# open-genome/dna

Measured on AMD Instinct MI355X. Metric: MLM sequences/sec, DNABERT-2-117M seq_len=512, at 1/2/4/8 MI355X, higher is better.
Workload: dtype bf16

## Files before the change

dna_amd/build.py:

```python
import argparse
import concurrent.futures as cf
import glob
import os
import shutil
import subprocess
import sys

HERE = os.path.dirname(os.path.abspath(__file__))
ROOT = os.path.dirname(HERE)
CSRC = os.path.join(HERE, "csrc")
INCLUDE = os.path.join(ROOT, "include")
BUILD = os.path.join(ROOT, "build", "native")
LIB = os.path.join(HERE, "lib", "libdna_amd.so")
ARCH = os.environ.get("DNA_AMD_ARCH", "gfx950")
HIPCC = os.environ.get("HIPCC", "/opt/rocm/bin/hipcc")

HIP_FLAGS = ["--offload-arch=" + ARCH, "-O3", "-fPIC", "-std=c++17", "-I", INCLUDE, "-I", CSRC,
             "-mllvm", "-amdgpu-mfma-vgpr-form",
             "-Wno-unused-result"]
FILE_FLAGS = {"attention.hip": ["-fno-honor-nans", "-fno-slp-vectorize"]}
for _item in filter(None, os.environ.get("DNA_AMD_FILE_FLAGS", "").split(";")):
    _f, _, _fl = _item.partition(":")
    FILE_FLAGS[_f.strip()] = FILE_FLAGS.get(_f.strip(), []) + _fl.split()
CXX_FLAGS = ["-O3", "-fPIC", "-std=c++17", "-pthread", "-I", INCLUDE, "-I", CSRC, "-Wall",
             "-Wno-unused-function"]


def _headers_mtime():
    hs = glob.glob(os.path.join(CSRC, "*.h")) + glob.glob(os.path.join(INCLUDE, "*.h"))
    return max((os.path.getmtime(h) for h in hs), default=0)


def _compile(src):
    obj = os.path.join(BUILD, os.path.basename(src) + ".o")
    if src.endswith(".hip"):
        cmd = [HIPCC] + HIP_FLAGS + FILE_FLAGS.get(os.path.basename(src), []) + ["-c", src, "-o", obj]
    else:
        cmd = ["g++"] + CXX_FLAGS + ["-c", src, "-o", obj]
    stamp = obj + ".cmd"
    line = " ".join(cmd)
    prev = open(stamp).read() if os.path.exists(stamp) else None
    if (os.path.exists(obj) and (prev == line or (prev is None and not os.environ.get("DNA_AMD_FILE_FLAGS")))
            and os.path.getmtime(obj) >= max(os.path.getmtime(src), _headers_mtime())):
        return obj, None
    r = subprocess.run(cmd, capture_output=True, text=True)
    if r.returncode != 0:
        return obj, f"$ {line}\n{r.stdout}\n{r.stderr}"
    with open(stamp, "w") as f:
        f.write(line)
    return obj, None


def _check_asm_lds_waits():
    obj = os.path.join(BUILD, "gemm.hip.o")
    stamp = obj + ".ldscheck"
    if not os.path.exists(obj) or (os.path.exists(stamp) and
                                   os.path.getmtime(stamp) >= os.path.getmtime(obj)):
        return
    sys.path.insert(0, os.path.join(ROOT, "scripts"))
    try:
        import check_lds_asm_waits as chk
    finally:
        sys.path.pop(0)
    n, bad = chk.check(chk.disassemble(obj))
    if bad or n == 0:
        os.remove(obj)
        raise RuntimeError(f"gemm.hip: {len(bad)} instructions touch an inline-asm LDS read's "
                           f"destination before its lgkmcnt(0) ({n} reads):\n" + "\n".join(bad[:20]))
    open(stamp, "w").close()


def build(verbose=False, jobs=None):
    os.makedirs(BUILD, exist_ok=True)
    os.makedirs(os.path.dirname(LIB), exist_ok=True)
    srcs = sorted(glob.glob(os.path.join(CSRC, "*.hip")) + glob.glob(os.path.join(CSRC, "*.cpp")))
    jobs = jobs or min(8, os.cpu_count() or 4)
    errors, objs = [], []
    with cf.ThreadPoolExecutor(jobs) as ex:
        for obj, err in ex.map(_compile, srcs):
            objs.append(obj)
            if err:
                errors.append(err)
    if errors:
        raise RuntimeError("native build failed:\n" + "\n".join(errors))
    _check_asm_lds_waits()
    if not os.path.exists(LIB) or os.path.getmtime(LIB) < max(os.path.getmtime(o) for o in objs):
        cmd = [HIPCC, "--offload-arch=" + ARCH, "-shared", "-fPIC", "-pthread", "-o", LIB] + objs
        r = subprocess.run(cmd, capture_output=True, text=True)
        if r.returncode != 0:
            raise RuntimeError(f"link failed:\n$ {' '.join(cmd)}\n{r.stdout}\n{r.stderr}")
        r = subprocess.run(["nm", "-D", "--undefined-only", LIB], capture_output=True, text=True)
        missing = [l.split()[-1] for l in r.stdout.splitlines() if "_ZN3dna" in l]
        if missing:
            os.remove(LIB)
            raise RuntimeError(f"libdna_amd.so has undefined own symbols: {missing}")
    if verbose:
        print(f"built {LIB}")
    return LIB


def main():
    ap = argparse.ArgumentParser()
    ap.add_argument("--clean", action="store_true")
    ap.add_argument("-j", type=int, default=None)
    args = ap.parse_args()
    if args.clean:
        shutil.rmtree(BUILD, ignore_errors=True)
        if os.path.exists(LIB):
            os.remove(LIB)
    build(verbose=True, jobs=args.j)


if __name__ == "__main__":
    sys.exit(main())
```

dna_amd/csrc/gemm.hip:

```cpp
#include <stdlib.h>

#include <type_traits>

#include "common.h"

namespace dna {
namespace gemm {

constexpr int BM = 256, BN = 256, BK = 64, NTHR = 512;
constexpr int HALF = 128 * BK * 2;
constexpr int LDS_BYTES = 8 * HALF;

enum Epi { EPI_BF16 = 0, EPI_F32 = 1, EPI_GEGLU = 2, EPI_GEGLU_BWD = 3, EPI_GELU_BWD = 4,
           EPI_BF16_GELU = 5 };

typedef __attribute__((address_space(3))) void lds_t;
typedef __attribute__((ext_vector_type(4))) short s16x4;

__device__ __forceinline__ int kswz(int r) { return (r >> 1) & 7; }
__device__ __forceinline__ int nswz(int r) { return ((r & 3) << 1) | (((r >> 3) & 1) << 3); }

__device__ __forceinline__ void glds16(const void* src, char* lds_base) {
  __builtin_amdgcn_global_load_lds(src, (lds_t*)lds_base, 16, 0, 0);
}

__device__ __forceinline__ int a_row(int lr, int mq) { return mq * 128 + lr; }
__device__ __forceinline__ int b_col(int lr, int nq) { return nq * 128 + lr; }

template <typename RowOf>
__device__ __forceinline__ void stage_k(const bf16* __restrict__ P, int ld, int k0, char* img,
                                        int wave, int lane, RowOf grow_of) {
#pragma unroll
  for (int p = 0; p < 2; ++p) {
    const int lr = p * 64 + wave * 8 + (lane >> 3);
    const int c = (lane & 7) ^ kswz(lr);
    glds16(P + (size_t)grow_of(lr) * ld + k0 + c * 8, img + (p * 64 + wave * 8) * 128);
  }
}

template <typename ColOf>
__device__ __forceinline__ void stage_n(const bf16* __restrict__ P, int ld, int k0, char* img,
                                        int wave, int lane, ColOf gcol_of) {
#pragma unroll
  for (int p = 0; p < 2; ++p) {
    const int r = p * 32 + wave * 4 + (lane >> 4);
    const int c = (lane & 15) ^ nswz(r);
    glds16(P + (size_t)(k0 + r) * ld + gcol_of(c * 8), img + (p * 32 + wave * 4) * 256);
  }
}

__device__ __forceinline__ bf16x8 read_k(const char* img, int lr, int chunk) {
  return *reinterpret_cast<const bf16x8*>(img + lr * 128 + ((chunk ^ kswz(lr)) << 4));
}

__device__ __forceinline__ bf16x4 tr_read(const char* p) {
  s16x4 v;
  const uint32_t a = (uint32_t)(uintptr_t)(const __attribute__((address_space(3))) char*)(p);
  asm volatile("ds_read_b64_tr_b16 %0, %1" : "=v"(v) : "v"(a) : "memory");
  return __builtin_bit_cast(bf16x4, v);
}

template <int OFF>
__device__ __forceinline__ bf16x4 tr_read_imm(uint32_t addr) {
  s16x4 v;
  asm volatile("ds_read_b64_tr_b16 %0, %1 offset:%2" : "=v"(v) : "v"(addr), "i"(OFF) : "memory");
  return __builtin_bit_cast(bf16x4, v);
}
__device__ __forceinline__ uint32_t lds_addr(const char* p) {
  return (uint32_t)(uintptr_t)(const __attribute__((address_space(3))) char*)(p);
}
__device__ __forceinline__ uint32_t read_n_lane_off(int c0, int lane) {
  const int i = lane & 15, kq = lane >> 4;
  const int r = kq * 8 + (i >> 2);
  const int col = c0 + 4 * (i & 3);
  return (uint32_t)(r * 256 + ((((col >> 3) ^ nswz(r)) << 4) + (col & 7) * 2));
}
__device__ __forceinline__ void read_n2(uint32_t addr, bf16x8& k0, bf16x8& k1) {
  const bf16x4 a = tr_read_imm<0>(addr), b = tr_read_imm<1024>(addr);
  const bf16x4 c = tr_read_imm<8192>(addr), d = tr_read_imm<9216>(addr);
  k0 = bf16x8{a[0], a[1], a[2], a[3], b[0], b[1], b[2], b[3]};
  k1 = bf16x8{c[0], c[1], c[2], c[3], d[0], d[1], d[2], d[3]};
}

__device__ __forceinline__ bf16x8 read_n(const char* img, int kbase, int c0, int lane) {
  const int i = lane & 15, kq = lane >> 4;
  const int r = kbase + kq * 8 + (i >> 2);
  const int col = c0 + 4 * (i & 3);
  const int off = (((col >> 3) ^ nswz(r)) << 4) + (col & 7) * 2;
  bf16x4 lo = tr_read(img + r * 256 + off);
  bf16x4 hi = tr_read(img + (r + 4) * 256 + off);
  return bf16x8{lo[0], lo[1], lo[2], lo[3], hi[0], hi[1], hi[2], hi[3]};
}

__device__ __forceinline__ f32x4 mfma(bf16x8 a, bf16x8 b, f32x4 c) {
  return __builtin_amdgcn_mfma_f32_16x16x32_bf16(a, b, c, 0, 0, 0);
}

struct Args {
  const bf16* A; int lda;
  const bf16* B; int ldb;
  void* C; int ldc;
  const float* bias;
  const bf16* g;
  bf16* aux;
  int M, N, K;
  int ksplit;
  int tilesM, tilesN, GM;
  int F;
  float p; uint32_t th; float ks; uint64_t seed, off;
  int rot;
  int dbg;
  int nt;
  int order;
};

__device__ __forceinline__ void tile_of(const Args& a, int& mt, int& nt) {
  const int nwg = gridDim.x, bid = blockIdx.x;
  const int xcd = bid & 7, q = nwg >> 3, rr = nwg & 7;
  const int L = (xcd < rr ? xcd * (q + 1) : rr * (q + 1) + (xcd - rr) * q) + (bid >> 3);
  const int width = a.GM * a.tilesN;
  const int grp = L / width, first = grp * a.GM;
  const int gsz = min(a.tilesM - first, a.GM);
  const int w = L - grp * width;
  mt = first + w % gsz;
  nt = w / gsz;
}

__device__ __forceinline__ void store_bf16x4(bf16* p, float v0, float v1, float v2, float v3) {
  *reinterpret_cast<bf16x4*>(p) = bf16x4{(bf16)v0, (bf16)v1, (bf16)v2, (bf16)v3};
}


typedef __attribute__((ext_vector_type(2))) unsigned u32x2;
typedef __attribute__((ext_vector_type(4))) unsigned u32x4;
constexpr uint32_t kOOB = 0x7FFFFFF0u;

__device__ __forceinline__ __amdgpu_buffer_rsrc_t out_rsrc(const void* base, uint32_t bytes) {
  return __builtin_amdgcn_make_buffer_rsrc(const_cast<void*>(base), (short)0, (int)bytes, 0x00020000);
}
__device__ __forceinline__ void store_b64(__amdgpu_buffer_rsrc_t r, uint32_t off, f32x4 v) {
  const bf16x4 h = bf16x4{(bf16)v[0], (bf16)v[1], (bf16)v[2], (bf16)v[3]};
  __builtin_amdgcn_raw_buffer_store_b64(__builtin_bit_cast(u32x2, h), r, off, 0, 0);
}
__device__ __forceinline__ void store_b64h(__amdgpu_buffer_rsrc_t r, uint32_t off, bf16x4 h) {
  __builtin_amdgcn_raw_buffer_store_b64(__builtin_bit_cast(u32x2, h), r, off, 0, 0);
}
__device__ __forceinline__ void store_b128(__amdgpu_buffer_rsrc_t r, uint32_t off, f32x4 v) {
  __builtin_amdgcn_raw_buffer_store_b128(__builtin_bit_cast(u32x4, v), r, off, 0, 0);
}
__device__ __forceinline__ void store_b128h(__amdgpu_buffer_rsrc_t r, uint32_t off, bf16x8 h) {
  __builtin_amdgcn_raw_buffer_store_b128(__builtin_bit_cast(u32x4, h), r, off, 0, 0);
}
__device__ __forceinline__ bf16x8 load_b128h(__amdgpu_buffer_rsrc_t r, uint32_t off) {
  return __builtin_bit_cast(bf16x8, __builtin_amdgcn_raw_buffer_load_b128(r, off, 0, 0));
}
__device__ float g_zero4[4];
__device__ __forceinline__ f32x4 bias4(const float* bias, int n, int limit) {
// ... 1472 lines not shown
    else if (abl == 1) hipLaunchKernelGGL((gemmp_kernel<EPI, 1>), dim3(G), dim3(NTHR), 0, s, a);
    else if (abl == 2) hipLaunchKernelGGL((gemmp_kernel<EPI, 2>), dim3(G), dim3(NTHR), 0, s, a);
    else if (abl == 3) hipLaunchKernelGGL((gemmp_kernel<EPI, 3>), dim3(G), dim3(NTHR), 0, s, a);
    else if (abl == 7) hipLaunchKernelGGL((gemmp_kernel<EPI, 7>), dim3(G), dim3(NTHR), 0, s, a);
    else if (abl == 8) hipLaunchKernelGGL((gemmp_kernel<EPI, 8>), dim3(G), dim3(NTHR), 0, s, a);
    else if (abl == 16) hipLaunchKernelGGL((gemmp_kernel<EPI, 16>), dim3(G), dim3(NTHR), 0, s, a);
    else if (abl == 32) hipLaunchKernelGGL((gemmp_kernel<EPI, 32>), dim3(G), dim3(NTHR), 0, s, a);
    else hipLaunchKernelGGL((gemmp_kernel<EPI>), dim3(G), dim3(NTHR), 0, s, a);
  }
  DNA_LAUNCH_CHECK(name);
  return DNA_OK;
}


inline int wgrad_chunks(int tiles, int KTtot, int G, double nk) {
  int best = 1;
  double best_cost = 1e30;
  for (int s = 1; s <= 64 && KTtot / s >= 4; ++s) {
    const int rounds = (tiles * s + G - 1) / G;
    const double cost = rounds * ((double)KTtot / s + 3.0) + s * nk * 8.0 / (6e12 * 1.6e-6);
    if (cost < best_cost - 1e-9) { best_cost = cost; best = s; }
  }
  return best;
}

inline int row_block(int M, int cap) {
  const int nblk = (M + cap - 1) / cap;
  const int per = (M + nblk - 1) / nblk;
  return (per + BM - 1) / BM * BM;
}

inline Args base_args() {
  Args a{};
  a.GM = 4;
  return a;
}

}
}

using namespace dna;
using namespace dna::gemm;

extern "C" int dna_linear_fwd(const void* x, const void* w, const float* bias, int M, int N, int K,
                              void* y, void* stream) {
  DNA_CHECK_ARG(x && w && y, "dna_linear_fwd: null pointer");
  DNA_CHECK_ARG(M >= 0 && N > 0 && K > 0, "dna_linear_fwd: bad shape");
  DNA_CHECK_ARG(K % BK == 0 && N % 8 == 0, "dna_linear_fwd: K %% 64 and N %% 8 required (K=%d N=%d)", K, N);
  if (M == 0) return DNA_OK;
  Args a = base_args();
  a.A = (const bf16*)x; a.lda = K;
  a.B = (const bf16*)w; a.ldb = K;
  a.C = y; a.ldc = N; a.bias = bias;
  a.M = M; a.N = N; a.K = K; a.ksplit = K;
  if (persistent_enabled() && N <= BIAS_LDS / 4 && N % BN == 0 && K >= 2 * BK &&
      (size_t)N * K * 2 < (1ull << 31)) {
    const size_t wide = (size_t)(K > N ? K : N) * 2;
    const int cap = (int)(((1ull << 31) - 1) / wide / BM * BM);
    if (cap >= BM) {
      const int mc = row_block(M, cap);
      for (int r0 = 0; r0 < M; r0 += mc) {
        Args c = a;
        c.A = a.A + (size_t)r0 * K;
        c.C = (bf16*)a.C + (size_t)r0 * N;
        c.M = M - r0 < mc ? M - r0 : mc;
        const int st = launchp<EPI_BF16>(c, as_stream(stream), "dna_linear_fwd");
        if (st != DNA_OK) return st;
      }
      return DNA_OK;
    }
  }
  return launch<true, true, EPI_BF16>(a, 1, as_stream(stream), "dna_linear_fwd");
}

extern "C" int dna_linear_gelu_fwd(const void* x, const void* w, const float* bias, int M, int N,
                                   int K, void* h, void* act, void* stream) {
  DNA_CHECK_ARG(x && w && h && act, "dna_linear_gelu_fwd: null pointer");
  DNA_CHECK_ARG(M >= 0 && N > 0 && K > 0, "dna_linear_gelu_fwd: bad shape");
  DNA_CHECK_ARG(N % BN == 0 && N <= BIAS_LDS / 4 && K % (2 * BK) == 0 &&
                    (size_t)N * K * 2 < (1ull << 31),
                "dna_linear_gelu_fwd: N %% 256 (<= %d) and K %% 128 required (N=%d K=%d)",
                BIAS_LDS / 4, N, K);
  if (M == 0) return DNA_OK;
  Args a = base_args();
  a.A = (const bf16*)x; a.lda = K;
  a.B = (const bf16*)w; a.ldb = K;
  a.C = h; a.ldc = N; a.bias = bias; a.aux = (bf16*)act;
  a.M = M; a.N = N; a.K = K; a.ksplit = K;
  const size_t wide = (size_t)(K > N ? K : N) * 2;
  const int cap = (int)(((1ull << 31) - 1) / wide / BM * BM);
  const int mc = row_block(M, cap);
  for (int r0 = 0; r0 < M; r0 += mc) {
    Args c = a;
    c.A = a.A + (size_t)r0 * K;
    c.C = (bf16*)a.C + (size_t)r0 * N;
    c.aux = a.aux + (size_t)r0 * N;
    c.M = M - r0 < mc ? M - r0 : mc;
    const int st = launchp<EPI_BF16_GELU>(c, as_stream(stream), "dna_linear_gelu_fwd");
    if (st != DNA_OK) return st;
  }
  return DNA_OK;
}

extern "C" int dna_linear_dgrad(const void* dy, const void* w, int M, int N, int K, void* dx,
                                void* stream) {
  DNA_CHECK_ARG(dy && w && dx, "dna_linear_dgrad: null pointer");
  DNA_CHECK_ARG(M >= 0 && N > 0 && K > 0, "dna_linear_dgrad: bad shape");
  DNA_CHECK_ARG(N % BK == 0 && K % 8 == 0, "dna_linear_dgrad: N %% 64 and K %% 8 required (N=%d K=%d)", N, K);
  if (M == 0) return DNA_OK;
  Args a = base_args();
  a.A = (const bf16*)dy; a.lda = N;
  a.B = (const bf16*)w; a.ldb = K;
  a.C = dx; a.ldc = K;
  a.M = M; a.N = K; a.K = N; a.ksplit = N;
  return launch<true, false, EPI_BF16>(a, 1, as_stream(stream), "dna_linear_dgrad");
}

extern "C" int dna_linear_wgrad(const void* dy, const void* x, int M, int N, int K, int splits,
                                float* partials, void* stream) {
  DNA_CHECK_ARG(dy && x && partials, "dna_linear_wgrad: null pointer");
  DNA_CHECK_ARG(M > 0 && N > 0 && K > 0 && splits > 0, "dna_linear_wgrad: bad shape");
  DNA_CHECK_ARG(M % (splits * BK) == 0, "dna_linear_wgrad: rows %d not a multiple of 64*splits", M);
  DNA_CHECK_ARG(N % 8 == 0 && K % 8 == 0, "dna_linear_wgrad: N, K %% 8 required");
  Args a = base_args();
  a.A = (const bf16*)dy; a.lda = N;
  a.B = (const bf16*)x; a.ldb = K;
  a.C = partials; a.ldc = K;
  a.M = N; a.N = K; a.K = M; a.ksplit = M / splits;
  a.GM = 2;
  return launch<false, false, EPI_F32>(a, splits, as_stream(stream), "dna_linear_wgrad");
}

extern "C" int dna_geglu_linear_fwd(const void* x, const void* w, const float* bias, int M, int F,
                                    int K, float p_drop, uint64_t seed, uint64_t offset, void* fac,
                                    void* out, void* stream) {
  DNA_CHECK_ARG(x && w && fac && out, "dna_geglu_linear_fwd: null pointer");
  void* g = fac;
  DNA_CHECK_ARG(M >= 0 && K % BK == 0 && F % (BN / 2) == 0,
                "dna_geglu_linear_fwd: K %% 64 and F %% 128 required (K=%d F=%d)", K, F);
  DNA_CHECK_ARG(p_drop >= 0.f && p_drop < 1.f, "dna_geglu_linear_fwd: bad p");
  if (M == 0) return DNA_OK;
  Args a = base_args();
  a.A = (const bf16*)x; a.lda = K;
  a.B = (const bf16*)w; a.ldb = K;
  a.C = g; a.ldc = 2 * F; a.bias = bias; a.aux = (bf16*)out;
  a.M = M; a.N = F; a.K = K; a.ksplit = K; a.F = F;
  a.p = p_drop; a.th = dropout_threshold16(p_drop); a.ks = 1.f / (1.f - p_drop);
  a.seed = seed; a.off = offset;
  if (persistent_enabled() && 2 * F <= BIAS_LDS / 4 && K >= 2 * BK && (size_t)2 * F * K * 2 < (1ull << 31)) {
    const size_t wide = (size_t)(K > 2 * F ? K : 2 * F) * 2;
    const int cap = (int)(((1ull << 31) - 1) / wide / BM * BM);
    if (cap >= BM) {
      const int mc = row_block(M, cap);
      for (int r0 = 0; r0 < M; r0 += mc) {
        Args c = a;
        c.A = a.A + (size_t)r0 * K;
        c.C = (bf16*)a.C + (size_t)r0 * 2 * F;
        c.aux = a.aux + (size_t)r0 * F;
        c.M = M - r0 < mc ? M - r0 : mc;
        c.off = a.off + (uint64_t)r0 * F / 8;
        const int st = launchp<EPI_GEGLU>(c, as_stream(stream), "dna_geglu_linear_fwd");
        if (st != DNA_OK) return st;
      }
      return DNA_OK;
    }
  }
  return launch<true, true, EPI_GEGLU>(a, 1, as_stream(stream), "dna_geglu_linear_fwd");
}

extern "C" int dna_geglu_linear_dgrad(const void* dy, const void* w, const void* fac, int M, int F,
                                      int N, void* dg, void* stream) {
  DNA_CHECK_ARG(dy && w && fac && dg, "dna_geglu_linear_dgrad: null pointer");
  const void* g = fac;
  DNA_CHECK_ARG(M >= 0 && N % BK == 0 && F % 8 == 0,
                "dna_geglu_linear_dgrad: hidden %% 64 and F %% 8 required (N=%d F=%d)", N, F);
  if (M == 0) return DNA_OK;
  Args a = base_args();
  a.A = (const bf16*)dy; a.lda = N;
  a.B = (const bf16*)w; a.ldb = F;
  a.C = nullptr; a.ldc = F; a.g = (const bf16*)g; a.aux = (bf16*)dg;
  a.M = M; a.N = F; a.K = N; a.ksplit = N; a.F = F;
  return launch<true, false, EPI_GEGLU_BWD>(a, 1, as_stream(stream), "dna_geglu_linear_dgrad");
}

extern "C" int dna_geglu_linear_dgrad_p(const void* dy, const void* wt, const void* fac, int M,
                                        int F, int N, void* dg, void* stream) {
  DNA_CHECK_ARG(dy && wt && fac && dg, "dna_geglu_linear_dgrad_p: null pointer");
  DNA_CHECK_ARG(M >= 0 && N % BK == 0 && (N / BK) % 2 == 0 && N >= 2 * BK && F % BN == 0,
                "dna_geglu_linear_dgrad_p: hidden %% 128 and F %% 256 required (N=%d F=%d)", N, F);
  const void* g = fac;
  DNA_CHECK_ARG((size_t)F * N * 2 < (1ull << 31), "dna_geglu_linear_dgrad_p: weight too large");
  if (M == 0) return DNA_OK;
  Args a = base_args();
  a.A = (const bf16*)dy; a.lda = N;
  a.B = (const bf16*)wt; a.ldb = N;
  a.C = nullptr; a.ldc = 2 * F; a.g = (const bf16*)g; a.aux = (bf16*)dg;
  a.N = F; a.K = N; a.ksplit = N; a.F = F;
  const char* ab = getenv("DNA_GEMM_ABL");
  const int abl = ab ? atoi(ab) : 0;
  a.tilesN = F / BN;
  a.GM = 8;
  if (const char* e = getenv("DNA_GEMM_GM")) a.GM = atoi(e);
  const size_t wide = (size_t)(N > 2 * F ? N : 2 * F) * 2;
  const int cap = (int)(((1ull << 31) - 1) / wide / BM * BM);
  DNA_CHECK_ARG(cap >= BM, "dna_geglu_linear_dgrad_p: rows of %zu bytes exceed 32-bit offsets", wide);
  const int mc = row_block(M, cap);
  for (int r0 = 0; r0 < M; r0 += mc) {
    Args c = a;
    c.A = a.A + (size_t)r0 * N;
    c.g = a.g + (size_t)r0 * 2 * F;
    c.aux = a.aux + (size_t)r0 * 2 * F;
    c.M = M - r0 < mc ? M - r0 : mc;
    c.tilesM = (c.M + BM - 1) / BM;
    const int U = c.tilesM * c.tilesN;
    int G = num_cus();
    G = U < G ? U : (G & ~7);
    if (abl == 128) hipLaunchKernelGGL((gemmp_kernel<EPI_GEGLU_BWD, 128, 2>), dim3(G), dim3(NTHR), 0, as_stream(stream), c);
    else hipLaunchKernelGGL((gemmp_kernel<EPI_GEGLU_BWD, 0, 2>), dim3(G), dim3(NTHR), 0, as_stream(stream), c);
    DNA_LAUNCH_CHECK("dna_geglu_linear_dgrad_p");
  }
  return DNA_OK;
}

extern "C" int dna_gelu_linear_dgrad_p(const void* dy, const void* wt, const void* h, int M, int F,
                                       int N, void* dh, void* stream) {
  DNA_CHECK_ARG(dy && wt && h && dh, "dna_gelu_linear_dgrad_p: null pointer");
  DNA_CHECK_ARG(M >= 0 && N % BK == 0 && (N / BK) % 2 == 0 && N >= 2 * BK && F % BN == 0,
                "dna_gelu_linear_dgrad_p: N %% 128 and F %% 256 required (N=%d F=%d)", N, F);
  DNA_CHECK_ARG((size_t)F * N * 2 < (1ull << 31), "dna_gelu_linear_dgrad_p: weight too large");
  if (M == 0) return DNA_OK;
  Args a = base_args();
  a.A = (const bf16*)dy; a.lda = N;
  a.B = (const bf16*)wt; a.ldb = N;
  a.C = nullptr; a.ldc = F; a.g = (const bf16*)h; a.aux = (bf16*)dh;
  a.N = F; a.K = N; a.ksplit = N; a.F = F;
  a.p = 0.f;
  a.tilesN = F / BN;
  a.GM = 8;
  if (const char* e = getenv("DNA_GEMM_GM")) a.GM = atoi(e);
  const size_t wide = (size_t)(N > F ? N : F) * 2;
  const int cap = (int)(((1ull << 31) - 1) / wide / BM * BM);
  DNA_CHECK_ARG(cap >= BM, "dna_gelu_linear_dgrad_p: rows of %zu bytes exceed 32-bit offsets", wide);
  const int mc = row_block(M, cap);
  for (int r0 = 0; r0 < M; r0 += mc) {
    Args c = a;
    c.A = a.A + (size_t)r0 * N;
    c.g = a.g + (size_t)r0 * F;
    c.aux = a.aux + (size_t)r0 * F;
    c.M = M - r0 < mc ? M - r0 : mc;
    c.tilesM = (c.M + BM - 1) / BM;
    const int U = c.tilesM * c.tilesN;
    int G = num_cus();
    G = U < G ? U : (G & ~7);
    hipLaunchKernelGGL((gemmp_kernel<EPI_GELU_BWD, 0, 2>), dim3(G), dim3(NTHR), 0, as_stream(stream), c);
    DNA_LAUNCH_CHECK("dna_gelu_linear_dgrad_p");
  }
  return DNA_OK;
}

extern "C" int dna_linear_wgrad_p_splits(int M, int N, int K) {
  if (M <= 0 || N % BM || K % BN) return 1;
  return wgrad_chunks((N / BM) * (K / BN), (M + BK - 1) / BK, num_cus() & ~7, (double)N * K);
}

extern "C" int dna_linear_wgrad_p(const void* dy, const void* x, int M, int N, int K, int splits,
                                  float* partials, void* stream) {
  DNA_CHECK_ARG(dy && x && partials, "dna_linear_wgrad_p: null pointer");
  DNA_CHECK_ARG(M > 0 && N % BM == 0 && K % BN == 0,
                "dna_linear_wgrad_p: N, K %% 256 required (N=%d K=%d)", N, K);
  const int KTtot = (M + BK - 1) / BK;
  DNA_CHECK_ARG(splits >= 1 && KTtot / splits >= 2, "dna_linear_wgrad_p: bad splits %d", splits);
  DNA_CHECK_ARG((size_t)((KTtot + splits - 1) / splits) * BK * (N > K ? N : K) * 2 < (1ull << 31) &&
                    (size_t)splits * N * K * 4 < (1ull << 32),
                "dna_linear_wgrad_p: chunks / partials too large for 32-bit buffer offsets");
  WArgs a{};
  a.dy = (const bf16*)dy; a.ldy = N;
  a.x = (const bf16*)x; a.ldx = K;
  a.part = partials;
  a.T = M; a.Nw = N; a.Kw = K;
  a.tilesM = N / BM; a.tilesN = K / BN; a.s = splits; a.KTtot = KTtot;
  const int U = a.tilesM * a.tilesN * splits;
  int G = num_cus() & ~7;
  G = U < G ? U : G;
  const char* ie = getenv("DNA_WGRAD_IMM");
  const int KTe = KTtot + (KTtot & 1);
  const bool pairs_ok = KTe / 2 / splits >= 1 &&
                        (size_t)((KTe / 2 + splits - 1) / splits) * 2 * BK * (N > K ? N : K) * 2 < (1ull << 31);
  if (gemm_sched() == 2 && pairs_ok && (!ie || atoi(ie) != 0)) {
    a.KTtot = KTe;
    hipLaunchKernelGGL((wgradp_kernel<true, 2>), dim3(G), dim3(NTHR), 0, as_stream(stream), a);
  }
  else if (gemm_sched() == 1 && (!ie || atoi(ie) != 0))
    hipLaunchKernelGGL((wgradp_kernel<true, 1>), dim3(G), dim3(NTHR), 0, as_stream(stream), a);
  else if (!ie || atoi(ie) != 0)
    hipLaunchKernelGGL(wgradp_kernel<true>, dim3(G), dim3(NTHR), 0, as_stream(stream), a);
  else
    hipLaunchKernelGGL(wgradp_kernel<false>, dim3(G), dim3(NTHR), 0, as_stream(stream), a);
  DNA_LAUNCH_CHECK("dna_linear_wgrad_p");
  return DNA_OK;
}
```

Baseline: 2521.

## Add dedicated persistent GEGLU forward kernel overlapping epilogue with next tile's MMA

Replaces the generic persistent GEMM path for the GEGLU forward linear with a new 256-thread, one-block-per-CU persistent kernel. It interleaves the previous tile's bias/GELU/dropout epilogue with the current tile's MFMA k-loop and keeps accumulators in AGPRs. The new file is compiled without the MFMA VGPR-form flag so the accumulators can live in AGPRs. The goal is to hide epilogue cost and memory stores behind matrix math. The trade-off is a large hand-scheduled kernel with tight register pressure, and it adds environment-variable debug knobs including one that skips the epilogue.

```diff
diff --git a/dna_amd/build.py b/dna_amd/build.py
--- a/dna_amd/build.py
+++ b/dna_amd/build.py
@@ -16,8 +16,9 @@
 HIPCC = os.environ.get("HIPCC", "/opt/rocm/bin/hipcc")
 
 HIP_FLAGS = ["--offload-arch=" + ARCH, "-O3", "-fPIC", "-std=c++17", "-I", INCLUDE, "-I", CSRC,
-             "-mllvm", "-amdgpu-mfma-vgpr-form",
              "-Wno-unused-result"]
+MFMA_VGPR_FORM = ["-mllvm", "-amdgpu-mfma-vgpr-form"]
+MFMA_AGPR_FILES = {"geglu_fwd_1w.hip"}
 FILE_FLAGS = {"attention.hip": ["-fno-honor-nans", "-fno-slp-vectorize"]}
 for _item in filter(None, os.environ.get("DNA_AMD_FILE_FLAGS", "").split(";")):
     _f, _, _fl = _item.partition(":")
@@ -34,7 +35,9 @@
 def _compile(src):
     obj = os.path.join(BUILD, os.path.basename(src) + ".o")
     if src.endswith(".hip"):
-        cmd = [HIPCC] + HIP_FLAGS + FILE_FLAGS.get(os.path.basename(src), []) + ["-c", src, "-o", obj]
+        name = os.path.basename(src)
+        cmd = ([HIPCC] + HIP_FLAGS + ([] if name in MFMA_AGPR_FILES else MFMA_VGPR_FORM) +
+               FILE_FLAGS.get(name, []) + ["-c", src, "-o", obj])
     else:
         cmd = ["g++"] + CXX_FLAGS + ["-c", src, "-o", obj]
     stamp = obj + ".cmd"
diff --git a/dna_amd/csrc/geglu_fwd_1w.h b/dna_amd/csrc/geglu_fwd_1w.h
--- /dev/null
+++ b/dna_amd/csrc/geglu_fwd_1w.h
@@ -0,0 +1,21 @@
+#pragma once
+#include "common.h"
+
+namespace dna {
+namespace gemm {
+
+struct Geglu1wArgs {
+  const bf16* A;
+  const bf16* B;
+  const float* bias;
+  bf16* fac;
+  bf16* out;
+  int M, F, K;
+  float p; uint32_t th; float ks; uint64_t seed, off;
+  int GM;
+};
+
+int launch_geglu_fwd_1w(const Geglu1wArgs& a, int grid_cap, bool epilogue, hipStream_t s);
+
+}
+}
diff --git a/dna_amd/csrc/geglu_fwd_1w.hip b/dna_amd/csrc/geglu_fwd_1w.hip
--- /dev/null
+++ b/dna_amd/csrc/geglu_fwd_1w.hip
@@ -0,0 +1,415 @@
+#include <stdlib.h>
+
+#include <type_traits>
+
+#include "geglu_fwd_1w.h"
+
+namespace dna {
+namespace geglu1w {
+
+using gemm::Geglu1wArgs;
+
+constexpr int BM = 256, BNH = 128, BK = 64, NTHR = 256;
+constexpr int HALF = 128 * BK * 2;
+constexpr int STAGE = 4 * HALF;
+constexpr int BIAS_LDS = 32 * 1024;
+constexpr int NS = 8;
+
+typedef __attribute__((address_space(3))) void lds_t;
+typedef __attribute__((ext_vector_type(2))) __bf16 bf16x2;
+typedef __attribute__((ext_vector_type(2))) unsigned u32x2;
+typedef __attribute__((ext_vector_type(4))) unsigned u32x4;
+
+__device__ __forceinline__ int kswz(int r) { return (r >> 1) & 7; }
+__device__ __forceinline__ uint32_t lds_addr(const void* p) {
+  return (uint32_t)(uintptr_t)(const __attribute__((address_space(3))) char*)(p);
+}
+__device__ __forceinline__ __amdgpu_buffer_rsrc_t rsrc(const void* base, size_t bytes) {
+  return __builtin_amdgcn_make_buffer_rsrc(const_cast<void*>(base), (short)0, (int)(uint32_t)bytes,
+                                           0x00020000);
+}
+__host__ __device__ constexpr int waitcnt_vm(int vm) {
+  return (vm & 0xF) | ((vm >> 4) << 14) | (0x7 << 4) | (0xF << 8);
+}
+__device__ __forceinline__ int xcd_remap(int b, int G) {
+  const int xcd = b & 7, q = G >> 3, r = G & 7;
+  return (xcd < r ? xcd * (q + 1) : r * (q + 1) + (xcd - r) * q) + (b >> 3);
+}
+
+#define DNA_BARRIER()                         \
+  do {                                        \
+    __builtin_amdgcn_sched_barrier(0);        \
+    __builtin_amdgcn_s_barrier();             \
+    asm volatile("" ::: "memory");            \
+    __builtin_amdgcn_sched_barrier(0);        \
+  } while (0)
+
+template <int V> using I = std::integral_constant<int, V>;
+
+template <int MODE>
+__global__ __launch_bounds__(NTHR, 1) void geglu_fwd_1w_kernel(Geglu1wArgs a) {
+  constexpr bool EPILOGUE = MODE != 0, DROP = MODE == 2;
+  __shared__ __attribute__((aligned(1024))) char smem[2 * STAGE + BIAS_LDS];
+  const int tid = threadIdx.x, lane = tid & 63;
+  const int wave = __builtin_amdgcn_readfirstlane(tid >> 6);
+  const int wr = wave >> 1, wc = wave & 1;
+  const int l16 = lane & 15, lq = lane >> 4;
+  const int G = gridDim.x;
+  const int tilesM = (a.M + BM - 1) / BM, tilesN = a.F / BNH;
+  const int U = tilesM * tilesN;
+  const int L = xcd_remap(blockIdx.x, G);
+  const int nb = L < U ? (U - L + G - 1) / G : 0;
+  if (nb == 0) return;
+  const int KT = a.K / BK;
+  const int K2 = a.K * 2;
+  float* bias_lds = reinterpret_cast<float*>(smem + 2 * STAGE);
+  for (int c = tid * 4; c < 2 * a.F; c += NTHR * 4)
+    *reinterpret_cast<f32x4*>(bias_lds + c) =
+        a.bias ? *reinterpret_cast<const f32x4*>(a.bias + c) : f32x4{0.f, 0.f, 0.f, 0.f};
+  __syncthreads();
+
+  const auto rA = rsrc(a.A, (size_t)a.M * K2);
+  const auto rB = rsrc(a.B, (size_t)2 * a.F * K2);
+  const auto rC = rsrc(a.fac, (size_t)a.M * a.F * 4);
+  const auto rAux = rsrc(a.out, (size_t)a.M * a.F * 2);
+
+  const uint32_t vo = (uint32_t)((wave * 8 + (lane >> 3)) * K2 + (((lane & 7) ^ kswz(wave * 8 + (lane >> 3))) << 4));
+  struct UC { int o[4], m0, n0; };
+  auto unit_at = [&](int i) {
+    const int u = L + i * G;
+    const int width = a.GM * tilesN;
+    const int grp = u / width, first = grp * a.GM;
+    const int gsz = min(tilesM - first, a.GM);
+    const int w = u - grp * width;
+    UC c;
+    c.m0 = (first + w % gsz) * BM;
+    c.n0 = (w / gsz) * BNH;
+    c.o[0] = __builtin_amdgcn_readfirstlane(c.m0 * K2);
+    c.o[1] = __builtin_amdgcn_readfirstlane((c.m0 + 128) * K2);
+    c.o[2] = __builtin_amdgcn_readfirstlane(c.n0 * K2);
+    c.o[3] = __builtin_amdgcn_readfirstlane((a.F + c.n0) * K2);
+    return c;
+  };
+  UC cur = unit_at(0), nxt = unit_at(nb > 1 ? 1 : 0), prv = cur;
+  int par = 0;
+  auto stage = [&](auto h_c, int k, int buf) {
+    constexpr int h = decltype(h_c)::value;
+    uint32_t toff = (uint32_t)(k < KT ? cur.o[h] + k * (BK * 2) : nxt.o[h] + (k - KT) * (BK * 2));
+    asm volatile("" : "+s"(toff));
+    char* d = smem + buf * STAGE + h * HALF + wave * 8 * 128;
+#pragma unroll
+    for (int p = 0; p < 4; ++p)
+      __builtin_amdgcn_raw_ptr_buffer_load_lds(h < 2 ? rA : rB, (lds_t*)(d + p * 32 * 128), 16,
+                                               vo + (toff + (uint32_t)(p * 32 * K2)), 0, 0, 0);
+  };
+
+  auto rd16 = [](uint32_t addr, auto off_c) {
+    constexpr int off = decltype(off_c)::value;
+    u32x4 r;
+    asm volatile("ds_read_b128 %0, %1 offset:%2" : "=v"(r) : "v"(addr), "i"(off) : "memory");
+    return r;
+  };
+  auto lgkm0 = [&]() {
+    asm volatile("s_waitcnt lgkmcnt(0)" ::: "memory");
+    __builtin_amdgcn_sched_barrier(0);
+  };
+  bf16x8 fa[2][4], fb[2][4];
+  auto settle = [&](bf16x8 (&f)[4]) {
+    asm volatile("s_waitcnt lgkmcnt(0)" : "+v"(f[0]), "+v"(f[1]), "+v"(f[2]), "+v"(f[3]) : : "memory");
+  };
+  auto settleA = [&](auto set_c) { settle(fa[decltype(set_c)::value]); };
+  auto settleB = [&](auto set_c) { settle(fb[decltype(set_c)::value]); };
+  const uint32_t sbase = lds_addr(smem);
+  uint32_t rbA[2], rbB[2];
+#pragma unroll
+  for (int kk = 0; kk < 2; ++kk) {
+    const uint32_t ch = (uint32_t)(((kk * 4 + lq) ^ kswz(l16)) << 4);
+    rbA[kk] = sbase + (wr * 64 + l16) * 128 + ch;
+    rbB[kk] = sbase + 2 * HALF + (wc * 64 + l16) * 128 + ch;
+  }
+  auto readA = [&](auto set_c, auto mq_c, auto kk_c) {
+    constexpr int s = decltype(set_c)::value, mq = decltype(mq_c)::value, kk = decltype(kk_c)::value;
+    fa[s][0] = __builtin_bit_cast(bf16x8, rd16(rbA[kk], I<mq * HALF>{}));
+    fa[s][1] = __builtin_bit_cast(bf16x8, rd16(rbA[kk], I<mq * HALF + 2048>{}));
+    fa[s][2] = __builtin_bit_cast(bf16x8, rd16(rbA[kk], I<mq * HALF + 4096>{}));
+    fa[s][3] = __builtin_bit_cast(bf16x8, rd16(rbA[kk], I<mq * HALF + 6144>{}));
+  };
+  auto readB = [&](auto set_c, auto nq_c, auto kk_c) {
+    constexpr int s = decltype(set_c)::value, nq = decltype(nq_c)::value, kk = decltype(kk_c)::value;
+    fb[s][0] = __builtin_bit_cast(bf16x8, rd16(rbB[kk], I<nq * HALF>{}));
+    fb[s][1] = __builtin_bit_cast(bf16x8, rd16(rbB[kk], I<nq * HALF + 2048>{}));
+    fb[s][2] = __builtin_bit_cast(bf16x8, rd16(rbB[kk], I<nq * HALF + 4096>{}));
+    fb[s][3] = __builtin_bit_cast(bf16x8, rd16(rbB[kk], I<nq * HALF + 6144>{}));
+  };
+
+  f32x4 acc[2][2][4][4];
+  auto mma = [&](auto as_c, auto bs_c, auto mq_c, auto nq_c, auto zi_c, auto h_c) {
+    constexpr int as = decltype(as_c)::value, bs = decltype(bs_c)::value;
+    constexpr int mq = decltype(mq_c)::value, nq = decltype(nq_c)::value, h = decltype(h_c)::value;
+    constexpr bool ZI = decltype(zi_c)::value;
+#pragma unroll
+    for (int i = 2 * h; i < 2 * h + 2; ++i)
+#pragma unroll
+      for (int j = 0; j < 4; ++j) {
+        f32x4& c = acc[mq][nq][i][j];
+        const bf16x8 wv = fb[bs][j], xv = fa[as][i];
+        if constexpr (ZI) asm volatile("v_mfma_f32_16x16x32_bf16 %0, %1, %2, 0" : "=a"(c) : "v"(wv), "v"(xv));
+        else asm volatile("v_mfma_f32_16x16x32_bf16 %0, %1, %2, %0" : "+a"(c) : "v"(wv), "v"(xv));
+      }
+  };
+
+  u32x4 hg1[16], hg2[16];
+  const int colq = wc * 64 + ((lq & 1) << 4) + ((lq & 2) << 2);
+  const uint32_t voG = (uint32_t)(((wr * 64 + l16) * 2 * a.F + colq) * 2);
+  const uint32_t voAx = (uint32_t)(((wr * 64 + l16) * a.F + colq) * 2);
+  auto swap8 = [&](f32x4 v0, f32x4 v1) __attribute__((always_inline)) {
+    u32x2 h0 = __builtin_bit_cast(u32x2, bf16x4{(bf16)v0[0], (bf16)v0[1], (bf16)v0[2], (bf16)v0[3]});
+    u32x2 h1 = __builtin_bit_cast(u32x2, bf16x4{(bf16)v1[0], (bf16)v1[1], (bf16)v1[2], (bf16)v1[3]});
+    const auto sx = __builtin_amdgcn_permlane16_swap(h0[0], h1[0], false, false);
+    const auto sy = __builtin_amdgcn_permlane16_swap(h0[1], h1[1], false, false);
+    return u32x4{sx[0], sy[0], sx[1], sy[1]};
+  };
+  auto pack = [&](const UC& c) __attribute__((always_inline)) {
+    asm volatile("s_nop 15\n\ts_nop 15" ::: "memory");
+    const uint32_t ba = lds_addr(bias_lds) + (uint32_t)((c.n0 + wc * 64 + 4 * lq) * 4);
+    const uint32_t bb = ba + (uint32_t)(a.F * 4);
+    auto slab = [&](auto jp_c) __attribute__((always_inline)) {
+      constexpr int jp = decltype(jp_c)::value;
+      const f32x4 b10 = __builtin_bit_cast(f32x4, rd16(ba, I<jp * 128>{}));
+      const f32x4 b11 = __builtin_bit_cast(f32x4, rd16(ba, I<jp * 128 + 64>{}));
+      const f32x4 b20 = __builtin_bit_cast(f32x4, rd16(bb, I<jp * 128>{}));
+      const f32x4 b21 = __builtin_bit_cast(f32x4, rd16(bb, I<jp * 128 + 64>{}));
+      lgkm0();
+#pragma unroll
+      for (int mq = 0; mq < 2; ++mq)
+#pragma unroll
+        for (int i = 0; i < 4; ++i) {
+          const int g = mq * 8 + i * 2 + jp;
+          hg1[g] = swap8(acc[mq][0][i][2 * jp] + b10, acc[mq][0][i][2 * jp + 1] + b11);
+          hg2[g] = swap8(acc[mq][1][i][2 * jp] + b20, acc[mq][1][i][2 * jp + 1] + b21);
+          __builtin_amdgcn_sched_barrier(0);
+        }
+    };
+    slab(I<0>{});
+    slab(I<1>{});
+    __builtin_amdgcn_sched_barrier(0);
+  };
+  struct EpS { uint4 r; u32x4 o, f1, f2; uint32_t w1, w2; float x, y1, y2; };
+  auto ep = [&](auto g_c, auto q_c, auto h_c, const UC& u, EpS& s) __attribute__((always_inline)) {
+    constexpr int g = decltype(g_c)::value, q = decltype(q_c)::value, h = decltype(h_c)::value;
+    constexpr int mq = g >> 3, i = (g >> 1) & 3, jp = g & 1;
+    int row = u.m0 + mq * 128 + i * 16;
+    asm volatile("" : "+s"(row));
+    if constexpr (q == 0 && h == 0 && DROP) {
+      int er = row + wr * 64 + l16;
+      asm volatile("" : "+v"(er));
+      const size_t e = (size_t)er * a.F + u.n0 + jp * 32 + colq;
+      s.r = dropout_draw8(a.seed, a.off, e >> 3);
+    } else if constexpr (q == 0 && h == 0) {
+      s.r = make_uint4(~0u, ~0u, ~0u, ~0u);
+    }
+    if constexpr (h == 0) {
+      s.w1 = hg1[g][q];
+      s.w2 = hg2[g][q];
+      asm volatile("" : "+v"(s.w1), "+v"(s.w2));
+    }
+    const bf16x2 h1 = __builtin_bit_cast(bf16x2, s.w1), h2 = __builtin_bit_cast(bf16x2, s.w2);
+    float x, y1, y2;
+    geglu_fwd_fac((float)h1[h], (float)h2[h], dropout_kept8(s.r, 2 * q + h, a.th), a.ks, x, y1, y2);
+    if constexpr (h == 0) {
+      s.x = x; s.y1 = y1; s.y2 = y2;
+    } else {
+      s.o[q] = __builtin_bit_cast(uint32_t, bf16x2{(bf16)s.x, (bf16)x});
+      s.f1[q] = __builtin_bit_cast(uint32_t, bf16x2{(bf16)s.y1, (bf16)y1});
+      s.f2[q] = __builtin_bit_cast(uint32_t, bf16x2{(bf16)s.y2, (bf16)y2});
+    }
+    if constexpr (q == 3 && h == 1) {
+      const uint32_t og = voG + (uint32_t)((row * 2 * a.F + u.n0 + jp * 32) * 2);
+      const uint32_t oa = voAx + (uint32_t)((row * a.F + u.n0 + jp * 32) * 2);
+      __builtin_amdgcn_raw_buffer_store_b128(s.f1, rC, og, 0, 0);
+      __builtin_amdgcn_raw_buffer_store_b128(s.f2, rC, og + a.F * 2, 0, 0);
+      __builtin_amdgcn_raw_buffer_store_b128(s.o, rAux, oa, 0, 0);
+    }
+  };
+  auto ep_group = [&](auto g_c, const UC& u) __attribute__((always_inline)) {
+    EpS s;
+    ep(g_c, I<0>{}, I<0>{}, u, s); ep(g_c, I<0>{}, I<1>{}, u, s);
+    ep(g_c, I<1>{}, I<0>{}, u, s); ep(g_c, I<1>{}, I<1>{}, u, s);
+    ep(g_c, I<2>{}, I<0>{}, u, s); ep(g_c, I<2>{}, I<1>{}, u, s);
+    ep(g_c, I<3>{}, I<0>{}, u, s); ep(g_c, I<3>{}, I<1>{}, u, s);
+    __builtin_amdgcn_sched_barrier(0);
+  };
+  auto bare_slice = [&](auto s_c, const UC& u) __attribute__((always_inline)) {
+    constexpr int sl = decltype(s_c)::value;
+    ep_group(I<2 * sl>{}, u);
+    ep_group(I<2 * sl + 1>{}, u);
+  };
+
+  using X = I<0>; using Y = I<1>; using P = I<0>; using Q = I<1>;
+  using K0 = I<0>; using K1 = I<1>;
+  using ZN = std::false_type;
+  auto step = [&](auto sl_c, auto zi_c, int k) __attribute__((always_inline)) {
+    constexpr int SL = decltype(sl_c)::value;
+    constexpr bool E = EPILOGUE && SL >= 0;
+    constexpr int GA = E ? 2 * SL : 0, GB = E ? 2 * SL + 1 : 0;
+    EpS s;
+    stage(I<3>{}, k + 1, par ^ 1);
+    stage(I<1>{}, k + 1, par ^ 1);
+    readB(Q{}, I<1>{}, K0{});
+    mma(X{}, P{}, I<0>{}, I<0>{}, zi_c, I<0>{});
+    if constexpr (E) ep(I<GA>{}, I<0>{}, I<0>{}, prv, s);
+    __builtin_amdgcn_sched_barrier(0);
+    mma(X{}, P{}, I<0>{}, I<0>{}, zi_c, I<1>{});
+    if constexpr (E) ep(I<GA>{}, I<0>{}, I<1>{}, prv, s);
+    settleB(Q{});
+    lgkm0();
+    readA(Y{}, I<1>{}, K0{});
+    mma(X{}, Q{}, I<0>{}, I<1>{}, zi_c, I<0>{});
+    if constexpr (E) ep(I<GA>{}, I<1>{}, I<0>{}, prv, s);
+    __builtin_amdgcn_sched_barrier(0);
+    mma(X{}, Q{}, I<0>{}, I<1>{}, zi_c, I<1>{});
+    if constexpr (E) ep(I<GA>{}, I<1>{}, I<1>{}, prv, s);
+    settleA(Y{});
+    lgkm0();
+    mma(Y{}, Q{}, I<1>{}, I<1>{}, zi_c, I<0>{});
+    if constexpr (E) ep(I<GA>{}, I<2>{}, I<0>{}, prv, s);
+    __builtin_amdgcn_sched_barrier(0);
+    mma(Y{}, Q{}, I<1>{}, I<1>{}, zi_c, I<1>{});
+    if constexpr (E) ep(I<GA>{}, I<2>{}, I<1>{}, prv, s);
+    __builtin_amdgcn_sched_barrier(0);
+    readA(X{}, I<0>{}, K1{});
+    readB(Q{}, I<0>{}, K1{});
+    mma(Y{}, P{}, I<1>{}, I<0>{}, zi_c, I<0>{});
+    if constexpr (E) ep(I<GA>{}, I<3>{}, I<0>{}, prv, s);
+    __builtin_amdgcn_sched_barrier(0);
+    mma(Y{}, P{}, I<1>{}, I<0>{}, zi_c, I<1>{});
+    if constexpr (E) ep(I<GA>{}, I<3>{}, I<1>{}, prv, s);
+    settleA(X{});
+    settleB(Q{});
+    lgkm0();
+    readB(P{}, I<1>{}, K1{});
+    mma(X{}, Q{}, I<0>{}, I<0>{}, ZN{}, I<0>{});
+    if constexpr (E) ep(I<GB>{}, I<0>{}, I<0>{}, prv, s);
+    __builtin_amdgcn_sched_barrier(0);
+    mma(X{}, Q{}, I<0>{}, I<0>{}, ZN{}, I<1>{});
+    if constexpr (E) ep(I<GB>{}, I<0>{}, I<1>{}, prv, s);
+    settleB(P{});
+    lgkm0();
+    readA(Y{}, I<1>{}, K1{});
+    mma(X{}, P{}, I<0>{}, I<1>{}, ZN{}, I<0>{});
+    if constexpr (E) ep(I<GB>{}, I<1>{}, I<0>{}, prv, s);
+    __builtin_amdgcn_sched_barrier(0);
+    mma(X{}, P{}, I<0>{}, I<1>{}, ZN{}, I<1>{});
+    if constexpr (E) ep(I<GB>{}, I<1>{}, I<1>{}, prv, s);
+    settleA(Y{});
+    lgkm0();
+    mma(Y{}, P{}, I<1>{}, I<1>{}, ZN{}, I<0>{});
+    if constexpr (E) ep(I<GB>{}, I<2>{}, I<0>{}, prv, s);
+    __builtin_amdgcn_sched_barrier(0);
+    mma(Y{}, P{}, I<1>{}, I<1>{}, ZN{}, I<1>{});
+    if constexpr (E) ep(I<GB>{}, I<2>{}, I<1>{}, prv, s);
+    __builtin_amdgcn_sched_barrier(0);
+    __builtin_amdgcn_s_waitcnt(waitcnt_vm(E ? 3 : 0));
+    DNA_BARRIER();
+    stage(I<0>{}, k + 2, par);
+    stage(I<2>{}, k + 2, par);
+    par ^= 1;
+    {
+      const uint32_t d = par ? (uint32_t)STAGE : (uint32_t)-STAGE;
+      rbA[0] += d; rbA[1] += d; rbB[0] += d; rbB[1] += d;
+    }
+    readA(X{}, I<0>{}, K0{});
+    readB(P{}, I<0>{}, K0{});
+    mma(Y{}, Q{}, I<1>{}, I<0>{}, ZN{}, I<0>{});
+    if constexpr (E) ep(I<GB>{}, I<3>{}, I<0>{}, prv, s);
+    __builtin_amdgcn_sched_barrier(0);
+    mma(Y{}, Q{}, I<1>{}, I<0>{}, ZN{}, I<1>{});
+    if constexpr (E) ep(I<GB>{}, I<3>{}, I<1>{}, prv, s);
+    settleA(X{});
+    settleB(P{});
+    lgkm0();
+  };
+
+  stage(I<0>{}, 0, 0);
+  stage(I<2>{}, 0, 0);
+  stage(I<3>{}, 0, 0);
+  stage(I<1>{}, 0, 0);
+  stage(I<0>{}, 1, 1);
+  stage(I<2>{}, 1, 1);
+  __builtin_amdgcn_s_waitcnt(waitcnt_vm(8));
+  DNA_BARRIER();
+  readA(X{}, I<0>{}, K0{});
+  readB(P{}, I<0>{}, K0{});
+  settleA(X{});
+  settleB(P{});
+  lgkm0();
+
+  using ZY = std::true_type;
+  for (int i = 0; i < nb; ++i) {
+    const bool have = EPILOGUE && i > 0;
+    if (have) {
+      step(I<0>{}, ZY{}, 0);
+      step(I<1>{}, ZN{}, 1);
+      if (KT > 2) step(I<2>{}, ZN{}, 2);
+      else bare_slice(I<2>{}, prv);
+      if (KT > 3) step(I<3>{}, ZN{}, 3);
+      else bare_slice(I<3>{}, prv);
+      if (KT > 4) step(I<4>{}, ZN{}, 4);
+      else bare_slice(I<4>{}, prv);
+      if (KT > 5) step(I<5>{}, ZN{}, 5);
+      else bare_slice(I<5>{}, prv);
+      if (KT > 6) step(I<6>{}, ZN{}, 6);
+      else bare_slice(I<6>{}, prv);
+      if (KT > 7) step(I<7>{}, ZN{}, 7);
+      else bare_slice(I<7>{}, prv);
+      for (int k = NS; k < KT; ++k) step(I<-1>{}, ZN{}, k);
+    } else {
+      step(I<-1>{}, ZY{}, 0);
+      for (int k = 1; k < KT; ++k) step(I<-1>{}, ZN{}, k);
+    }
+    if constexpr (EPILOGUE) {
+      pack(cur);
+    }
+    prv = cur;
+    cur = nxt;
+    nxt = unit_at(i + 2 < nb ? i + 2 : nb - 1);
+  }
+  if constexpr (EPILOGUE) {
+    bare_slice(I<0>{}, prv);
+    bare_slice(I<1>{}, prv);
+    bare_slice(I<2>{}, prv);
+    bare_slice(I<3>{}, prv);
+    bare_slice(I<4>{}, prv);
+    bare_slice(I<5>{}, prv);
+    bare_slice(I<6>{}, prv);
+    bare_slice(I<7>{}, prv);
+  } else {
+#pragma unroll
+    for (int q = 0; q < 4; ++q)
+#pragma unroll
+      for (int i = 0; i < 4; ++i)
+#pragma unroll
+        for (int j = 0; j < 4; ++j) asm volatile("" ::"a"(acc[q >> 1][q & 1][i][j]));
+  }
+  asm volatile("s_waitcnt vmcnt(0)" ::: "memory");
+}
+
+}
+
+namespace gemm {
+
+int launch_geglu_fwd_1w(const Geglu1wArgs& a, int grid_cap, bool epilogue, hipStream_t s) {
+  const int U = ((a.M + geglu1w::BM - 1) / geglu1w::BM) * (a.F / geglu1w::BNH);
+  const int G = U < grid_cap ? U : (grid_cap & ~7);
+  if (!epilogue)
+    hipLaunchKernelGGL((geglu1w::geglu_fwd_1w_kernel<0>), dim3(G), dim3(geglu1w::NTHR), 0, s, a);
+  else if (a.p > 0.f)
+    hipLaunchKernelGGL((geglu1w::geglu_fwd_1w_kernel<2>), dim3(G), dim3(geglu1w::NTHR), 0, s, a);
+  else
+    hipLaunchKernelGGL((geglu1w::geglu_fwd_1w_kernel<1>), dim3(G), dim3(geglu1w::NTHR), 0, s, a);
+  DNA_LAUNCH_CHECK("dna_geglu_linear_fwd");
+  return DNA_OK;
+}
+
+}
+}
diff --git a/dna_amd/csrc/gemm.hip b/dna_amd/csrc/gemm.hip
--- a/dna_amd/csrc/gemm.hip
+++ b/dna_amd/csrc/gemm.hip
@@ -3,6 +3,7 @@
 #include <type_traits>
 
 #include "common.h"
+#include "geglu_fwd_1w.h"
 
 namespace dna {
 namespace gemm {
@@ -1781,14 +1782,23 @@
     const int cap = (int)(((1ull << 31) - 1) / wide / BM * BM);
     if (cap >= BM) {
       const int mc = row_block(M, cap);
+      Geglu1wArgs w{};
+      w.B = a.B; w.bias = bias; w.F = F; w.K = K;
+      w.p = a.p; w.th = a.th; w.ks = a.ks; w.seed = seed;
+      w.GM = a.GM;
+      if (const char* e = getenv("DNA_GEMM_GM")) w.GM = atoi(e);
+      if (w.GM <= 0) w.GM = 8;
+      int G = num_cus();
+      if (const char* e = getenv("DNA_GEMM_GRID")) G = atoi(e);
+      const char* ab = getenv("DNA_GEMM_ABL");
+      const bool epilogue = !(ab && atoi(ab) == 64);
       for (int r0 = 0; r0 < M; r0 += mc) {
-        Args c = a;
-        c.A = a.A + (size_t)r0 * K;
-        c.C = (bf16*)a.C + (size_t)r0 * 2 * F;
-        c.aux = a.aux + (size_t)r0 * F;
-        c.M = M - r0 < mc ? M - r0 : mc;
-        c.off = a.off + (uint64_t)r0 * F / 8;
-        const int st = launchp<EPI_GEGLU>(c, as_stream(stream), "dna_geglu_linear_fwd");
+        w.A = a.A + (size_t)r0 * K;
+        w.fac = (bf16*)a.C + (size_t)r0 * 2 * F;
+        w.out = a.aux + (size_t)r0 * F;
+        w.M = M - r0 < mc ? M - r0 : mc;
+        w.off = a.off + (uint64_t)r0 * F / 8;
+        const int st = launch_geglu_fwd_1w(w, G, epilogue, as_stream(stream));
         if (st != DNA_OK) return st;
       }
       return DNA_OK;
```

New measurement: 2383. 0.945x the previous value.
